# harmony-one/harmony

Hardware: AMD Instinct MI355X
Metric: BLS12-381 aggregate-verifies/sec (committee=4096) (higher is better)
Workload: dtype u64; 1 GPU; config2: committee=4096 masked aggregate + pairing verify, batch=262144/step, masks Bernoulli(0.9) seed 42, 48B staking commit payloads; parallelism=dp1 (per-shard replicas, no collective)

## Files before the change

harmony_amd/core.py:

```python
import ctypes
import os

_DIR = os.path.dirname(os.path.abspath(__file__))
_SO = os.environ.get("HBLS_SO", os.path.join(_DIR, "libhbls.so"))

HBLS_OK = 1
HBLS_FALSE = 0
HBLS_ERR = -1
HBLS_ERR_NOGPU = -2
HBLS_ERR_BADINPUT = -3
HBLS_NOQUORUM = -4
NOQUORUM = HBLS_NOQUORUM
TWO_THIRDS_DEC = 666666666666666667


class HblsError(RuntimeError):
    pass


class NoGpuError(HblsError):
    pass


class BadInputError(HblsError, ValueError):
# ... 40 lines not shown
        ctypes.c_char_p, ctypes.c_char_p, ctypes.c_size_t, ctypes.c_size_t,
        ctypes.POINTER(ctypes.c_int32)]
    lib.hbls_stream_create.restype = ctypes.c_void_p
    lib.hbls_stream_create.argtypes = [ctypes.c_void_p, ctypes.c_int]
    lib.hbls_stream_free.argtypes = [ctypes.c_void_p]
    lib.hbls_stream_set_rounds.argtypes = [
        ctypes.c_void_p, ctypes.POINTER(ctypes.c_uint32), ctypes.c_int,
        ctypes.c_char_p, ctypes.c_size_t]
    lib.hbls_stream_process.argtypes = [
        ctypes.c_void_p, ctypes.POINTER(ctypes.c_uint32),
        ctypes.POINTER(ctypes.c_uint32), ctypes.c_char_p,
        ctypes.POINTER(ctypes.c_uint32), ctypes.c_int,
        ctypes.c_size_t, ctypes.POINTER(ctypes.c_int32)]
    lib.hbls_stream_check.argtypes = [
        ctypes.c_void_p, ctypes.POINTER(ctypes.c_uint32), ctypes.c_int,
        ctypes.POINTER(ctypes.c_int32)]
    lib.hbls_stream_check_submit.argtypes = [
        ctypes.c_void_p, ctypes.POINTER(ctypes.c_uint32), ctypes.c_int]
    lib.hbls_stream_check_poll.argtypes = [
        ctypes.c_void_p, ctypes.POINTER(ctypes.c_int32)]
    lib.hbls_stream_get.argtypes = [ctypes.c_void_p, ctypes.c_uint32,
                                    ctypes.c_char_p, ctypes.c_char_p]
    lib.hbls_stream_set_verify_mode.argtypes = [ctypes.c_void_p, ctypes.c_int]
    lib.hbls_batch_verify_votes_grouped.argtypes = [
        ctypes.c_void_p, ctypes.POINTER(ctypes.c_uint32),
        ctypes.POINTER(ctypes.c_uint32), ctypes.c_char_p, ctypes.c_char_p,
        ctypes.c_size_t, ctypes.c_size_t, ctypes.c_size_t,
        ctypes.POINTER(ctypes.c_int32)]
    lib.hbls_vote_key_sums.argtypes = [
        ctypes.c_void_p, ctypes.POINTER(ctypes.c_uint32),
        ctypes.POINTER(ctypes.c_uint32), ctypes.c_size_t, ctypes.c_char_p,
        ctypes.POINTER(ctypes.c_int32)]
    lib.hbls_batch_verify_votes_multi.argtypes = [
        ctypes.c_void_p, ctypes.POINTER(ctypes.c_uint32),
        ctypes.POINTER(ctypes.c_uint32), ctypes.c_char_p, ctypes.c_char_p,
        ctypes.c_size_t, ctypes.c_size_t, ctypes.POINTER(ctypes.c_int32)]
    lib.hbls_stream_process_multi.argtypes = [
        ctypes.c_void_p, ctypes.POINTER(ctypes.c_uint32),
        ctypes.POINTER(ctypes.c_uint32), ctypes.POINTER(ctypes.c_uint32),
        ctypes.c_char_p, ctypes.POINTER(ctypes.c_uint32), ctypes.c_int,
        ctypes.c_size_t, ctypes.POINTER(ctypes.c_int32)]
    lib.hbls_rlc_last_stats.argtypes = [ctypes.POINTER(ctypes.c_uint32)]
    lib.hbls_rlc_last_stats.restype = None
    lib.hbls_set_agg_verify_mode.argtypes = [ctypes.c_int]
    lib.hbls_set_aggrlc_threshold.argtypes = [ctypes.c_int]
    lib.hbls_set_aggrlc_threshold.restype = None
    lib.hbls_aggrlc_last_stats.argtypes = [ctypes.POINTER(ctypes.c_uint32)]
    lib.hbls_aggrlc_last_stats.restype = None
    lib.hbls_set_aggrlc_final.argtypes = [ctypes.c_int]
    lib.hbls_aggrlc_final_selftest.argtypes = [ctypes.c_int]
    lib.hbls_set_aggrlc_sigleg.argtypes = [ctypes.c_int]
    lib.hbls_set_aggrlc_early.argtypes = [ctypes.c_int]
    lib.hbls_set_aggrlc_chunkleg.argtypes = [ctypes.c_int]
    lib.hbls_aggrlc_probe.argtypes = [ctypes.c_int, ctypes.c_char_p, ctypes.c_size_t,
                                      ctypes.c_char_p]
    lib.hbls_last_host_ns.restype = ctypes.c_uint64
    lib.hbls_last_host_ns.argtypes = [ctypes.c_int]
    u64p, u32p, i32p = (ctypes.POINTER(t) for t in
                        (ctypes.c_uint64, ctypes.c_uint32, ctypes.c_int32))
    lib.hbls_committee_set_quorum.argtypes = [ctypes.c_void_p, u64p, ctypes.c_uint64]
    lib.hbls_mask_power.argtypes = [ctypes.c_void_p, ctypes.c_char_p, ctypes.c_size_t,
                                    u64p, u32p]
    lib.hbls_agg_verify_quorum.argtypes = lib.hbls_agg_verify.argtypes
    lib.hbls_batch_agg_verify_quorum.argtypes = lib.hbls_batch_agg_verify.argtypes
    lib.hbls_batch_seal_verify_quorum.argtypes = lib.hbls_batch_seal_verify.argtypes
    lib.hbls_stream_power.argtypes = [ctypes.c_void_p, u32p, ctypes.c_int,
                                      u64p, u32p, i32p]
    lib.hbls_last_stage_ns.argtypes = [ctypes.c_int]
    lib.hbls_copy_bench_ns.restype = ctypes.c_uint64
    lib.hbls_copy_bench_ns.argtypes = [ctypes.c_size_t]
    lib.hbls_fpmul_bench_waves.restype = ctypes.c_double
    lib.hbls_fpmul_bench_waves.argtypes = [ctypes.c_int, ctypes.c_int]
    lib.hbls_coop_selftest.restype = ctypes.c_int
    lib.hbls_fpmul_asm_check.restype = ctypes.c_longlong
    lib.hbls_arith_probe.argtypes = [ctypes.c_int, ctypes.c_char_p, ctypes.c_size_t,
                                     ctypes.c_char_p, i32p]
    lib.hbls_arith_probe_op_name.argtypes = [ctypes.c_int]
    lib.hbls_arith_probe_op_name.restype = ctypes.c_char_p
    if hasattr(lib, "hbls_ctxset_create"):
        lib.hbls_ctxset_create.restype = ctypes.c_void_p
        lib.hbls_ctxset_create.argtypes = [ctypes.POINTER(ctypes.c_void_p), ctypes.c_size_t]
        lib.hbls_ctxset_free.argtypes = [ctypes.c_void_p]
        lib.hbls_ctxset_free.restype = None
        lib.hbls_ctxset_size.argtypes = [ctypes.c_void_p]
        lib.hbls_ctxset_size.restype = ctypes.c_size_t
        lib.hbls_batch_seal_verify_ctx.argtypes = [
            ctypes.c_void_p, u32p, ctypes.c_char_p, u32p, ctypes.c_char_p, u32p,
            ctypes.c_size_t, ctypes.c_int, i32p]
        lib.hbls_ctx_mask_sums.argtypes = [
            ctypes.c_void_p, u32p, ctypes.c_char_p, u32p, ctypes.c_size_t,
            ctypes.c_char_p, u64p, u32p, i32p]
    return lib


_lib = _load()


def _check(rc, what):
    if rc == HBLS_ERR_NOGPU:
        raise NoGpuError(f"{what}: no AMD GPU available (product path requires gfx950)")
    if rc == HBLS_ERR_BADINPUT:
        raise BadInputError(f"{what}: bad input")
    if rc < 0:
        raise HblsError(f"{what}: error {rc}")
    return rc

# ... 24 lines not shown

def set_coop_threshold(n: int):
    _lib.hbls_set_coop_threshold(n)


def rlc_chunk_size() -> int:
    return _lib.hbls_rlc_chunk_size()


def rlc_last_stats():
    out = (ctypes.c_uint32 * 4)()
    _lib.hbls_rlc_last_stats(out)
    return list(out)


def set_agg_verify_mode(mode: int):
    _check(_lib.hbls_set_agg_verify_mode(mode), "set_agg_verify_mode")


def set_aggrlc_threshold(n: int):
    _lib.hbls_set_aggrlc_threshold(n)


def aggrlc_chunk_size() -> int:
    return _lib.hbls_aggrlc_chunk_size()


def aggrlc_last_stats():
    out = (ctypes.c_uint32 * 3)()
    _lib.hbls_aggrlc_last_stats(out)
    return list(out)


def set_aggrlc_final(kernel: int):
    _check(_lib.hbls_set_aggrlc_final(kernel), "set_aggrlc_final")


def aggrlc_final_selftest(nchunks: int) -> int:
    return _check(_lib.hbls_aggrlc_final_selftest(nchunks), "aggrlc_final_selftest")


def set_aggrlc_sigleg(leg: int):
    _check(_lib.hbls_set_aggrlc_sigleg(leg), "set_aggrlc_sigleg")


def set_aggrlc_early(early: int):
    _check(_lib.hbls_set_aggrlc_early(early), "set_aggrlc_early")


def set_aggrlc_chunkleg(kernel: int):
    _check(_lib.hbls_set_aggrlc_chunkleg(kernel), "set_aggrlc_chunkleg")


AGGRLC_PROBE_OPS = {"g1_mul64w": (0, 3 * 48 + 8, 3 * 48),
                    "g2_mul64w": (1, 6 * 48 + 8, 6 * 48),
                    "miller1_fe": (2, 6 * 48, 12 * 48)}


def aggrlc_probe(name: str, data: bytes, n_items: int) -> bytes:
    op, in_b, out_b = AGGRLC_PROBE_OPS[name]
    if len(data) != n_items * in_b:
        raise ValueError("aggrlc_probe: operand size")
    out = ctypes.create_string_buffer(max(1, n_items * out_b))
    _check(_lib.hbls_aggrlc_probe(op, data, n_items, out), "aggrlc_probe")
    return out.raw[:n_items * out_b]


def last_host_ns(i: int) -> int:
    return _lib.hbls_last_host_ns(i)


def pk_from_sk(sk32: bytes) -> bytes:
    out = ctypes.create_string_buffer(48)
    _check(_lib.hbls_pk_from_sk(sk32, out), "pk_from_sk")
    return out.raw


def batch_pk_from_sk(sks: bytes, batch: int) -> bytes:
    out = ctypes.create_string_buffer(48 * batch)
    _check(_lib.hbls_batch_pk_from_sk(sks, batch, out), "batch_pk_from_sk")
    return out.raw


def sign_hash(sk32: bytes, msg: bytes) -> bytes:
    out = ctypes.create_string_buffer(96)
    _check(_lib.hbls_sign_hash(sk32, msg, len(msg), out), "sign_hash")
    return out.raw


def batch_sign(sks: bytes, msgs: bytes, mlen: int, batch: int) -> bytes:
    out = ctypes.create_string_buffer(96 * batch)
    _check(_lib.hbls_batch_sign(sks, msgs, mlen, batch, out), "batch_sign")
    return out.raw


def hash_to_g2(msg: bytes) -> bytes:
    out = ctypes.create_string_buffer(96)
    _check(_lib.hbls_hash_to_g2(msg, len(msg), out), "hash_to_g2")
    return out.raw


def batch_hash_to_g2(msgs: bytes, mlen: int, batch: int) -> bytes:
    out = ctypes.create_string_buffer(96 * batch)
    _check(_lib.hbls_batch_hash_to_g2(msgs, mlen, batch, out), "batch_hash_to_g2")
    return out.raw


def verify_hash(pk48: bytes, sig96: bytes, msg: bytes) -> bool:
    rc = _lib.hbls_verify_hash(pk48, sig96, msg, len(msg))
# ... 456 lines not shown
```

harmony_amd/csrc/hbls_aggrlc.inc:

```

#define AGGRLC_CHUNK 64
#define AGGRLC_WINDOWS 8


DEV void aggrlc_recode64(uint64_t k, uint64_t &mag, uint32_t &neg, uint32_t &top) {
    uint32_t c = 0;
    mag = 0; neg = 0;
#pragma unroll
    for (int j = 0; j < 16; j++) {
        uint32_t v = ((uint32_t)(k >> (4 * j)) & 15u) + c;
        uint32_t nx = j < 15 ? ((uint32_t)(k >> (4 * j + 4)) & 15u) : 0u;
        c = (v > 8u || (v == 8u && nx >= 8u)) ? 1u : 0u;
        uint32_t m = c ? 16u - v : v;
        mag |= (uint64_t)m << (4 * j);
        neg |= (c && m) ? (1u << j) : 0u;
    }
    top = c;
}

DEVN void g1_mul64w(g1_t &r, const g1_t &p, uint64_t k) {
    g1_t tab[8];
    tab[0] = p;
    g1_dbl(tab[1], tab[0]);
    g1_add(tab[2], tab[1], tab[0]);
// ... 196 lines not shown
__global__ void k_aggrlc_miller1(const g1_t *aggpubs, const g2_t *hms,
                                 const uint64_t *scalars, const g2aff_t *S,
                                 const int32_t *sflag, fp12_t *F, int32_t *elig,
                                 int32_t *results, int batch, int nchunks,
                                 int32_t *dirty) {
    size_t i = (size_t)blockIdx.x * blockDim.x + threadIdx.x;
    if (i >= (size_t)batch + (size_t)nchunks) return;
    fp12_t f;
    g2aff_t Q;
    g1aff_t P;
    bool run = false;
    if (i < (size_t)batch) {
        if (HOISTED) {
            int32_t e = elig[i];
            if (e == AGGRLC_ELIG_OPEN) {
                results[i] = g1_is_inf(aggpubs[i]) ? 1 : 0;
                elig[i] = 0;
            } else if (e == 1 && g1_is_inf(aggpubs[i])) {
                results[i] = 0;
                elig[i] = 0;
                dirty[i / AGGRLC_CHUNK] = 1;
            }
        }
        if (elig[i] == 1) {
            uint64_t r = scalars[i];
            if (r == 0) r = 1;
            g1_t A;
            g1_mul64w(A, aggpubs[i], r);
            if (g1_is_inf(A)) {
                elig[i] = 2; results[i] = 0;
            } else {
                g1_to_affine(P, A);
                g2_t hmc = hms[i];
                g2_to_affine(Q, hmc);
                run = true;
            }
        }
    } else {
        size_t c = i - (size_t)batch;
        if (sflag[c]) {
            Q = S[c];
            fp_load(P.x, BLS_G1_X);
            fp_t gy;
            fp_load(gy, BLS_G1_Y);
            fp_neg(P.y, gy);
            run = true;
        }
    }
    if (run) miller_loop1_h(f, Q, P);
    else fp12_one(f);
    F[i] = f;
}

__global__ void k_aggrlc_chunkleg(const g2aff_t *S, const int32_t *sflag,
                                  const int32_t *dirty, fp12_t *FX, int nchunks) {
    int c = blockIdx.x * blockDim.x + threadIdx.x;
    if (c >= nchunks) return;
    if (dirty && !dirty[c]) return;
    fp12_t f;
    if (sflag[c]) {
        g2aff_t Q = S[c];
        g1aff_t P;
        fp_load(P.x, BLS_G1_X);
        fp_t gy;
        fp_load(gy, BLS_G1_Y);
        fp_neg(P.y, gy);
        miller_loop1_h(f, Q, P);
    } else {
        fp12_one(f);
    }
    FX[c] = f;
}

DEVN void cv_miller1(lds_fp2 *A, int q) {
    if (q == 0) {
        lds_st(A + CV_T1, lds_ld(A + CV_Q1));
        lds_st(A + (CV_T1 + 1), lds_ld(A + (CV_Q1 + 1)));
        fp2_t one; fp_one(one.a); fp_zero(one.b);
        lds_st(A + (CV_T1 + 2), one);
    }
    __syncthreads();
    cv_fp12_set_one(A, q, CV_F0);
    int cur = CV_F0, oth = CV_F1;
    for (int bit = 62; bit >= 0; bit--) {
        cv_fp12_sqr(A, q, oth, cur);
        { int s = cur; cur = oth; oth = s; }
        cv_ml_dbl_step(A, q, CV_T1, CV_PP);
        cv_fp12_mul_line(A, q, oth, cur);
        { int s = cur; cur = oth; oth = s; }
        if ((BLS_U >> bit) & 1) {
            cv_ml_add_step(A, q, CV_T1, CV_Q1, CV_PP);
            cv_fp12_mul_line(A, q, oth, cur);
            { int s = cur; cur = oth; oth = s; }
        }
    }
    if (cur != CV_F0) cv_fp12_copy(A, q, CV_F0, cur);
}

template <int ITEMS>
__global__ void __launch_bounds__(ITEMS * CV_LANES) k_aggrlc_chunkleg_coop(
        const g2aff_t *S, const int32_t *sflag, fp12_t *FX, int nchunks) {
    __shared__ uint64_t arena[ITEMS][CV_STRIDE64];
    __shared__ int32_t pre[ITEMS];
    const int sub = threadIdx.x / CV_LANES;
    const int q = threadIdx.x % CV_LANES;
    const int c = blockIdx.x * ITEMS + sub;
// ... 150 lines not shown
    return HBLS_OK;
}
extern "C" void hbls_set_aggrlc_threshold(int n) {
    g_aggrlc_threshold = n < 0 ? AGGRLC_DEFAULT_THRESHOLD : n;
}

#define AGGRLC_FINAL_DEFAULT 16
static int g_aggrlc_final = -2;
static int aggrlc_final_kernel(void) {
    if (g_aggrlc_final == -2) {
        const char *e = getenv("HBLS_AGGRLC_FINAL");
        int k = e ? atoi(e) : AGGRLC_FINAL_DEFAULT;
        g_aggrlc_final = (k == 0 || k == 8 || k == 16) ? k : AGGRLC_FINAL_DEFAULT;
    }
    return g_aggrlc_final;
}
extern "C" int hbls_set_aggrlc_final(int kernel) {
    if (kernel == -1) kernel = AGGRLC_FINAL_DEFAULT;
    if (kernel != 0 && kernel != 8 && kernel != 16) return HBLS_ERR_BADINPUT;
    g_aggrlc_final = kernel;
    return HBLS_OK;
}
#define AGGRLC_SIGLEG_MIN_BATCH 16384
static int g_aggrlc_sigleg = -2;
static int aggrlc_sigleg(size_t batch) {
    if (g_aggrlc_sigleg == -2) {
        const char *e = getenv("HBLS_AGGRLC_SIGLEG");
        int k = e ? atoi(e) : -1;
        g_aggrlc_sigleg = (k == 0 || k == 1) ? k : -1;
    }
    if (g_aggrlc_sigleg >= 0) return g_aggrlc_sigleg;
    return batch >= AGGRLC_SIGLEG_MIN_BATCH ? 1 : 0;
}
extern "C" int hbls_set_aggrlc_sigleg(int leg) {
    if (leg < -1 || leg > 1) return HBLS_ERR_BADINPUT;
    g_aggrlc_sigleg = leg;
    return HBLS_OK;
}

#define AGGRLC_EARLY_MIN_BATCH 262144
static int g_aggrlc_early = -2;
static int aggrlc_early(size_t batch) {
    if (g_aggrlc_early == -2) {
        const char *e = getenv("HBLS_AGGRLC_EARLY");
        int k = e ? atoi(e) : -1;
        g_aggrlc_early = (k == 0 || k == 1) ? k : -1;
    }
    if (g_aggrlc_early >= 0) return g_aggrlc_early;
    return batch >= AGGRLC_EARLY_MIN_BATCH ? 1 : 0;
}
extern "C" int hbls_set_aggrlc_early(int early) {
    if (early < -1 || early > 1) return HBLS_ERR_BADINPUT;
    g_aggrlc_early = early;
    return HBLS_OK;
}

#define AGGRLC_CHUNKLEG_DEFAULT 16
static int g_aggrlc_chunkleg = -2;
static int aggrlc_chunkleg_kernel(void) {
    if (g_aggrlc_chunkleg == -2) {
        const char *e = getenv("HBLS_AGGRLC_CHUNKLEG");
        int k = e ? atoi(e) : AGGRLC_CHUNKLEG_DEFAULT;
        g_aggrlc_chunkleg = (k == 0 || k == 16) ? k : AGGRLC_CHUNKLEG_DEFAULT;
    }
    return g_aggrlc_chunkleg;
}
extern "C" int hbls_set_aggrlc_chunkleg(int kernel) {
    if (kernel == -1) kernel = AGGRLC_CHUNKLEG_DEFAULT;
    if (kernel != 0 && kernel != 16) return HBLS_ERR_BADINPUT;
    g_aggrlc_chunkleg = kernel;
    return HBLS_OK;
}

static hipStream_t g_aggrlc_side_stream = nullptr;
static std::once_flag g_aggrlc_side_flag;
static hipStream_t aggrlc_side_stream(void) {
    std::call_once(g_aggrlc_side_flag, [] {
        hipStream_t s = nullptr;
        int least = 0, greatest = 0;
        if (hipDeviceGetStreamPriorityRange(&least, &greatest) != hipSuccess) {
            (void)hipGetLastError();
            greatest = 0;
        }
        if (hipStreamCreateWithPriority(&s, hipStreamNonBlocking, greatest) == hipSuccess)
            g_aggrlc_side_stream = s;
        else
            (void)hipGetLastError();
    });
    return g_aggrlc_side_stream;
}

struct AggrlcEarly {
    size_t batch, nc;
    std::vector<uint64_t> scalars;
    DevBuf dsc, dB, dS, dFX, delig, dflag;
    EventSet<5> ev;
    bool launched = false;
    AggrlcEarly(size_t b, size_t n)
        : batch(b), nc(n), scalars(b), dsc(b * 8), dB(b * sizeof(g2_t)),
          dS(n * sizeof(g2aff_t)), dFX(n * sizeof(fp12_t)), delig(b * 4), dflag(2 * n * 4) {}
    bool ok() const {
        return !dsc.err && !dB.err && !dS.err && !dFX.err && !delig.err && !dflag.err &&
               ev.err == hipSuccess;
    }
    int32_t *sflag() const { return dflag.as<int32_t>(); }
    int32_t *dirty() const { return dflag.as<int32_t>() + nc; }
// ... 114 lines not shown
    std::vector<int32_t> v(3 * nc);
    HIP_OK(hipMemcpy(v.data(), dv.p, 3 * nc * 4, hipMemcpyDeviceToHost));
    int zeros = 0, ones = 0;
    for (size_t c = 0; c < nc; c++) {
        int kind = (int)(c % 8);
        int want = (kind == 1 || kind == 2 || kind == 3) ? 1 : 0;
        if (v[c] != want) return HBLS_ERR;
        if (v[c]) ones++; else zeros++;
    }
    if (nc >= 2 && (!zeros || !ones)) return HBLS_ERR;
    int diff = 0;
    for (size_t c = 0; c < nc; c++)
        if (v[nc + c] != v[c] || v[2 * nc + c] != v[c]) diff++;
    return diff;
}

static g1aff_t *g_aggrlc_gtab = nullptr;
static int aggrlc_init_tables(void) {
    if (g_aggrlc_gtab) return HBLS_OK;
    const size_t m = AGGRLC_WINDOWS * 255;
    DevBuf dp2(64 * sizeof(g1aff_t)), dwj(m * sizeof(g1_t)), dwi(m);
    g1aff_t *d_gt = nullptr;
    if (dp2.err || dwj.err || dwi.err) return HBLS_ERR;
    HIP_OK(hipMalloc(&d_gt, m * sizeof(g1aff_t)));
    hipLaunchKernelGGL(k_aggrlc_pow2, dim3(1), dim3(64), 0, 0, dp2.as<g1aff_t>());
    hipLaunchKernelGGL(k_wtab_build_jac, dim3(1), dim3(64), 0, 0,
                       dp2.as<g1aff_t>(), 64, dwj.as<g1_t>(), AGGRLC_WINDOWS);
    hipLaunchKernelGGL(k_wtab_to_affine, dim3((int)((m + 255) / 256)), dim3(256), 0, 0,
                       dwj.as<g1_t>(), d_gt, dwi.as<uint8_t>(), m);
    std::vector<uint8_t> winf(m);
    bool ok = hipDeviceSynchronize() == hipSuccess &&
              hipMemcpy(winf.data(), dwi.p, m, hipMemcpyDeviceToHost) == hipSuccess;
    for (size_t k = 0; ok && k < m; k++)
        if (winf[k]) ok = false;
    if (!ok) { hipFree(d_gt); return HBLS_ERR; }
    g_aggrlc_gtab = d_gt;
    return HBLS_OK;
}

static bool aggrlc_wanted(size_t batch) {
    int m = agg_verify_mode();
    if (m == 0 || !g_aggrlc_gtab) return false;
    if (batch > RLC_MAX_ITEMS || (long long)batch < (long long)g_aggrlc_threshold) return false;
    if (m == 1) return true;
    return (int)batch > coop_threshold() && rf_mode() == 0 && !use_batch_affine();
}

static int aggrlc_verify(const g1_t *d_agg, const g2_t *d_hm, const g2aff_t *d_saff,
                         const int32_t *d_sflags, const int32_t *d_hok,
                         int32_t *d_res, size_t batch, AggrlcEarly *early) {
    size_t nc = (batch + AGGRLC_CHUNK - 1) / AGGRLC_CHUNK;
    const int leg = early ? 1 : aggrlc_sigleg(batch);
    const size_t nx = (leg && !early) ? nc : 0;
    std::vector<uint64_t> scalars(early ? 0 : batch);
    if (!early && !rlc_draw_scalars(scalars.data(), batch)) return AGGRLC_FALLBACK;
    FreeClock fclk;
    uint64_t t_alloc = host_now_ns();
    const size_t f_bytes = (batch + nx) * sizeof(fp12_t);
    const size_t b_bytes = nx ? batch * sizeof(g2_t) : 0;
    DevBuf dsc(early ? 0 : batch * 8), dF(f_bytes + b_bytes + nx * sizeof(g2aff_t));
    DevBuf delig(early ? 0 : batch * 4);
    DevBuf dFC(nc * sizeof(fp12_t)), dcs((3 * nc + nx) * 4);
    g_host_ns[0] += host_now_ns() - t_alloc;
    FreeClockArm farm(fclk);
    if (dsc.err || dF.err || delig.err || dFC.err || dcs.err) {
        (void)hipGetLastError();
        return AGGRLC_FALLBACK;
    }
    fp12_t *d_F = dF.as<fp12_t>();
    g2_t *d_B = (g2_t *)((uint8_t *)dF.p + f_bytes);
    g2aff_t *d_S = (g2aff_t *)((uint8_t *)dF.p + f_bytes + b_bytes);
    const uint64_t *d_sc = early ? early->dsc.as<uint64_t>() : dsc.as<uint64_t>();
    int32_t *d_elig = early ? early->delig.as<int32_t>() : delig.as<int32_t>();
    EventSet<1> up;
    if (up.err != hipSuccess) return HBLS_ERR;
    if (!early) HIP_OK(upload_then_wait(dsc.p, scalars.data(), batch * 8, up[0]));
    int32_t *d_ccnt = dcs.as<int32_t>(), *d_cforce = d_ccnt + nc, *d_verdict = d_cforce + nc;
    int32_t *d_sf = d_verdict + nc;
    EventSet<5> ev;
    if (ev.err != hipSuccess) return HBLS_ERR;
    (void)hipEventRecord(ev[0], 0);
    if (leg && !early) {
        hipLaunchKernelGGL(k_aggrlc_sigscale<false>, dim3((uint32_t)((batch + 63) / 64)), dim3(64),
                           0, 0, d_agg, d_saff, d_sflags, d_hok, d_sc, d_B,
                           d_elig, d_res, (int)batch);
        hipLaunchKernelGGL(k_aggrlc_sigsum<false>, dim3((uint32_t)nc), dim3(AGGRLC_CHUNK), 0, 0,
                           d_B, (int)batch, (int)nc, d_S, d_sf,
                           (const int32_t *)nullptr, (const int32_t *)nullptr);
    }
    (void)hipEventRecord(ev[1], 0);
    if (early) {
        hipLaunchKernelGGL(k_aggrlc_miller1<true>, dim3((uint32_t)((batch + 63) / 64)), dim3(64),
                           0, 0, d_agg, d_hm, d_sc, early->dS.as<g2aff_t>(), early->sflag(), d_F,
                           d_elig, d_res, (int)batch, 0, early->dirty());
        (void)hipStreamWaitEvent(0, early->ev[3], 0);
        hipLaunchKernelGGL(k_aggrlc_sigsum<true>, dim3((uint32_t)nc), dim3(AGGRLC_CHUNK), 0, 0,
                           early->dB.as<g2_t>(), (int)batch, (int)nc, early->dS.as<g2aff_t>(),
                           early->sflag(), d_elig, early->dirty());
        hipLaunchKernelGGL(k_aggrlc_chunkleg, dim3((uint32_t)((nc + 63) / 64)), dim3(64), 0, 0,
                           early->dS.as<g2aff_t>(), early->sflag(), early->dirty(),
                           early->dFX.as<fp12_t>(), (int)nc);
    } else if (leg) {
        hipLaunchKernelGGL(k_aggrlc_miller1<false>, dim3((uint32_t)((batch + nc + 63) / 64)),
                           dim3(64), 0, 0, d_agg, d_hm, d_sc, d_S, d_sf, d_F,
                           d_elig, d_res, (int)batch, (int)nc, (int32_t *)nullptr);
    } else {
        hipLaunchKernelGGL(k_aggrlc_miller, dim3((uint32_t)((batch + 63) / 64)), dim3(64), 0, 0,
                           d_agg, d_hm, d_saff, d_sflags, d_hok, d_sc,
                           g_aggrlc_gtab, d_F, d_elig, d_res, (int)batch);
    }
    (void)hipEventRecord(ev[2], 0);
    hipLaunchKernelGGL(k_aggrlc_chunk_prod, dim3((uint32_t)nc), dim3(AGGRLC_CHUNK), 0, 0,
                       d_F, d_elig, (int)batch, (int)nc,
                       dFC.as<fp12_t>(), d_ccnt, d_cforce,
                       early ? early->dFX.as<fp12_t>()
                             : leg ? d_F + batch : (const fp12_t *)nullptr);
    (void)hipEventRecord(ev[3], 0);
    launch_aggrlc_final(aggrlc_final_kernel(), dFC.as<fp12_t>(), d_ccnt, d_cforce,
                        d_verdict, (int)nc);
    (void)hipEventRecord(ev[4], 0);
    std::vector<int32_t> hc(3 * nc);
    hipError_t e = hipMemcpy(hc.data(), dcs.p, 3 * nc * 4, hipMemcpyDeviceToHost);
    if (e == hipSuccess) e = hipGetLastError();
    for (int i = 0; i < 4; i++) {
        float ms = 0;
        if (e == hipSuccess && (i || (leg && !early)))
            (void)hipEventElapsedTime(&ms, ev[i], ev[i + 1]);
        g_stage_ns[i ? 3 + i : 7] = (uint64_t)(ms * 1e6);
    }
    if (early && e == hipSuccess) {
        float ms = 0;
        (void)hipEventElapsedTime(&ms, early->ev[0], early->ev[1]);
        g_stage_ns[7] = (uint64_t)(ms * 1e6);
        ms = 0;
        (void)hipEventElapsedTime(&ms, early->ev[2], early->ev[3]);
        g_stage_ns[8] = (uint64_t)(ms * 1e6);
    }
    HIP_OK(e);

    std::vector<uint32_t> failed;
    for (size_t c = 0; c < nc; c++) {
        if (hc[c] <= 0) continue;
        g_aggrlc_stats[0]++;
        if (hc[2 * nc + c] == 1) continue;
        g_aggrlc_stats[1]++;
        failed.push_back((uint32_t)c);
    }
    if (failed.empty()) return HBLS_OK;

    std::vector<int32_t> helig(batch);
    HIP_OK(hipMemcpy(helig.data(), d_elig, batch * 4, hipMemcpyDeviceToHost));
    std::vector<uint32_t> sel;
    for (uint32_t c : failed)
        for (size_t i = (size_t)c * AGGRLC_CHUNK;
             i < batch && i < ((size_t)c + 1) * AGGRLC_CHUNK; i++)
            if (helig[i]) sel.push_back((uint32_t)i);
    size_t ns = sel.size();
    g_aggrlc_stats[2] = (uint32_t)ns;
    if (!ns) return HBLS_OK;
    DevBuf dsel(ns * 4);
    if (dsel.err) return HBLS_ERR;
    HIP_OK(hipMemcpy(dsel.p, sel.data(), ns * 4, hipMemcpyHostToDevice));
    hipLaunchKernelGGL(k_verify_sel, dim3((uint32_t)((ns + 63) / 64)), dim3(64), 0, 0,
                       dsel.as<uint32_t>(), (int)ns, d_agg, d_hm, d_saff, d_sflags, d_hok,
                       d_res, (int)batch);
    HIP_OK(hipGetLastError());
    return HBLS_OK;
}

enum { AGGRLC_PROBE_G1_MUL64W = 0, AGGRLC_PROBE_G2_MUL64W = 1, AGGRLC_PROBE_MILLER1_FE = 2,
       AGGRLC_PROBE_N_OPS = 3 };
#define AGGRLC_PROBE_MAX_ITEMS 4096
__global__ void k_aggrlc_probe(int op, const uint64_t *in, int in_w, uint64_t *out, int out_w,
                               int n) {
    int j = blockIdx.x * blockDim.x + threadIdx.x;
    if (j >= n) return;
    const uint64_t *src = in + (size_t)j * in_w;
    uint64_t *dst = out + (size_t)j * out_w;
    union { uint64_t w[72]; g1_t g1; g2_t g2; g2aff_t q; fp12_t f; } a, o;
    for (int i = 0; i < in_w && i < 72; i++) a.w[i] = src[i];
    if (op == AGGRLC_PROBE_G1_MUL64W) {
        g1_mul64w(o.g1, a.g1, src[18]);
    } else if (op == AGGRLC_PROBE_G2_MUL64W) {
        g2_mul64w(o.g2, a.g2, src[36]);
    } else {
        g1aff_t p;
        for (int k = 0; k < 6; k++) { p.x.l[k] = src[24 + k]; p.y.l[k] = src[30 + k]; }
        fp12_t f;
        miller_loop1_h(f, a.q, p);
        fp12_conj(f, f);
        final_exp(o.f, f);
    }
    for (int i = 0; i < out_w; i++) dst[i] = o.w[i];
}
static bool probe_limbs_lt_p(const uint8_t *b);
extern "C" int hbls_aggrlc_probe(int op, const uint8_t *in, size_t n_items, uint8_t *out) {
    if (op < 0 || op >= AGGRLC_PROBE_N_OPS) return HBLS_ERR_BADINPUT;
    if (!in || !out || n_items == 0 || n_items > AGGRLC_PROBE_MAX_ITEMS)
        return HBLS_ERR_BADINPUT;
    const int n_fp = op == AGGRLC_PROBE_G1_MUL64W ? 3 : 6;
    const int in_w = n_fp * 6 + (op == AGGRLC_PROBE_MILLER1_FE ? 0 : 1);
    const int out_w = op == AGGRLC_PROBE_G1_MUL64W ? 18 : op == AGGRLC_PROBE_G2_MUL64W ? 36 : 72;
    for (size_t j = 0; j < n_items; j++)
        for (int i = 0; i < n_fp; i++)
            if (!probe_limbs_lt_p(in + j * (size_t)in_w * 8 + 48 * i)) return HBLS_ERR_BADINPUT;
    int rc = require_gpu();
    if (rc != HBLS_OK) return rc;
    DevBuf din(n_items * in_w * 8), dout(n_items * out_w * 8);
    if (din.err || dout.err) return HBLS_ERR;
    HIP_OK(hipMemcpy(din.p, in, n_items * in_w * 8, hipMemcpyHostToDevice));
    hipLaunchKernelGGL(k_aggrlc_probe, dim3((uint32_t)((n_items + 63) / 64)), dim3(64), 0, 0,
                       op, din.as<uint64_t>(), in_w, dout.as<uint64_t>(), out_w, (int)n_items);
    HIP_OK(hipGetLastError());
    HIP_OK(hipDeviceSynchronize());
    HIP_OK(hipMemcpy(out, dout.p, n_items * out_w * 8, hipMemcpyDeviceToHost));
    return HBLS_OK;
}
```

harmony_amd/csrc/hbls_dev.hip:

```cpp
#include <hip/hip_runtime.h>
#include <stdint.h>
#include <string.h>
#include <stdio.h>
#include <stdlib.h>
#include "../../oracle/bls_consts.h"
#include "../../include/hbls.h"

typedef unsigned __int128 u128;

#define DEV __device__ __forceinline__
#define DEVN __device__ __noinline__

struct fp_t { uint64_t l[6]; };
struct fp2_t { fp_t a, b; };

DEV bool fp_is_zero(const fp_t &x) {
    return (x.l[0] | x.l[1] | x.l[2] | x.l[3] | x.l[4] | x.l[5]) == 0;
}
DEV bool fp_eq(const fp_t &x, const fp_t &y) {
    uint64_t d = 0;
#pragma unroll
    for (int i = 0; i < 6; i++) d |= x.l[i] ^ y.l[i];
    return d == 0;
}
// ... 1088 lines not shown
    fp2_dbl(E, E); fp2_dbl(E, E);
    fp2_dbl(t, E); fp2_add(E, E, t);
    fp2_dbl(t, E); fp2_add(F, E, t);
    fp2_add(G, B, F);
    fp2_half(G, G);
    fp2_add(H, T.y, T.z);
    fp2_sqr(H, H);
    fp2_add(t, B, C);
    fp2_sub(H, H, t);
    fp2_sqr(XX, T.x);
    fp2_mul_fp(t, H, Pa.y);
    fp2_mul_xi(c0, t);
    fp2_sub(c3, B, E);
    fp2_dbl(t, XX); fp2_add(t, t, XX);
    fp2_mul_fp(t, t, Pa.x);
    fp2_neg(c5, t);
    fp2_sub(t, B, F);
    fp2_mul(T.x, A, t);
    fp2_sqr(t, G);
    fp2_sqr(t2, E);
    fp2_dbl(G, t2); fp2_add(t2, t2, G);
    fp2_sub(T.y, t, t2);
    fp2_mul(T.z, B, H);
}
DEVN void ml_add_step_h(g2_t &T, const g2aff_t &Q, const g1aff_t &Pa,
                        fp2_t &c0, fp2_t &c3, fp2_t &c5) {
    fp2_t th, la, C, D, E, F, G, H, t, t2;
    fp2_mul(t, Q.y, T.z);
    fp2_sub(th, T.y, t);
    fp2_mul(t, Q.x, T.z);
    fp2_sub(la, T.x, t);
    fp2_mul_fp(t, la, Pa.y);
    fp2_mul_xi(c0, t);
    fp2_mul(t, Q.x, th);
    fp2_mul(t2, Q.y, la);
    fp2_sub(c3, t, t2);
    fp2_mul_fp(t, th, Pa.x);
    fp2_neg(c5, t);
    fp2_sqr(C, th);
    fp2_sqr(D, la);
    fp2_mul(E, la, D);
    fp2_mul(F, T.z, C);
    fp2_mul(G, T.x, D);
    fp2_add(H, E, F);
    fp2_dbl(t, G);
    fp2_sub(H, H, t);
    fp2_mul(T.x, la, H);
    fp2_sub(t, G, H);
    fp2_mul(t, th, t);
    fp2_mul(t2, E, T.y);
    fp2_sub(T.y, t, t2);
    fp2_mul(T.z, T.z, E);
}
DEVN void fp12_mul_line2(fp12_t &f, const fp2_t &a0, const fp2_t &a3, const fp2_t &a5,
                         const fp2_t &b0, const fp2_t &b3, const fp2_t &b5) {
    fp6_t m0, t0, t1, fs, tt, vt1;
    fp2_t p00, p33, p55, x, y, s, u, q1, q2, q3;
    fp2_mul(p00, a0, b0);
    fp2_mul(p33, a3, b3);
    fp2_mul(p55, a5, b5);
    fp2_add(s, a3, a5);
    fp2_add(u, b3, b5);
    fp2_mul(q1, s, u);
    fp2_sub(q1, q1, p33);
    fp2_sub(q1, q1, p55);
    fp2_mul_xi(m0.c1, q1);
    fp2_mul_xi(s, p33);
    fp2_add(m0.c0, p00, s);
    fp2_mul_xi(m0.c2, p55);
    fp2_add(s, a0, a3);
    fp2_add(u, b0, b3);
    fp2_mul(x, s, u);
    fp2_sub(x, x, p00);
    fp2_sub(x, x, p33);
    fp2_add(s, a0, a5);
    fp2_add(u, b0, b5);
    fp2_mul(y, s, u);
    fp2_sub(y, y, p00);
    fp2_sub(y, y, p55);
    fp6_mul(t0, f.c0, m0);
    {
        const fp2_t &g0 = f.c1.c0, &g1 = f.c1.c1, &g2 = f.c1.c2;
        fp2_mul(q1, g1, x);
        fp2_mul(q2, g2, y);
        fp2_add(s, g1, g2);
        fp2_add(u, x, y);
        fp2_mul(q3, s, u);
        fp2_sub(q3, q3, q1);
        fp2_sub(q3, q3, q2);
        fp2_mul_xi(t1.c0, q3);
        fp2_mul(s, g0, x);
        fp2_mul_xi(u, q2);
        fp2_add(t1.c1, s, u);
        fp2_mul(s, g0, y);
        fp2_add(t1.c2, s, q1);
    }
    fp6_add(fs, f.c0, f.c1);
    fp2_add(m0.c1, m0.c1, x);
    fp2_add(m0.c2, m0.c2, y);
    fp6_mul(tt, fs, m0);
    fp6_sub(tt, tt, t0);
    fp6_sub(tt, tt, t1);
    fp6_mul_v(vt1, t1);
    fp6_add(f.c0, t0, vt1);
    f.c1 = tt;
}
// ... 2988 lines not shown
```

include/hbls.h:

```cpp
#ifndef HBLS_H
#define HBLS_H

#include <stddef.h>
#include <stdint.h>

#ifdef __cplusplus
extern "C" {
#endif

enum {
    HBLS_OK = 1,
    HBLS_FALSE = 0,
    HBLS_ERR = -1,
    HBLS_ERR_NOGPU = -2,
    HBLS_ERR_BADINPUT = -3,
    HBLS_NOQUORUM = -4,
};

#define HBLS_TWO_THIRDS_DEC 666666666666666667ULL

int hbls_init(int device);

int hbls_device_count(void);

// ... 104 lines not shown
                               const uint8_t *msgs,  const uint32_t *msg_off,
                               size_t batch, int quorum, int32_t *results);

int hbls_ctx_mask_sums(const hbls_ctxset_t *s, const uint32_t *ctx_idx,
                       const uint8_t *bitmaps, const uint32_t *bm_off, size_t batch,
                       uint8_t *out48s, uint64_t *power_out, uint32_t *count_out,
                       int32_t *ok);

int hbls_g2_aggregate(const uint8_t *sigs96, size_t n, uint8_t out96[96]);

typedef struct hbls_stream hbls_stream_t;
hbls_stream_t *hbls_stream_create(const hbls_committee_t *c, int max_rounds);
void hbls_stream_free(hbls_stream_t *s);
int hbls_stream_set_rounds(hbls_stream_t *s, const uint32_t *slots, int k,
                           const uint8_t *payloads, size_t payload_len);
int hbls_stream_process(hbls_stream_t *s, const uint32_t *key_idx,
                        const uint32_t *round_idx, const uint8_t *sigs96,
                        const uint32_t *active_slots, int n_active,
                        size_t batch, int32_t *results);
int hbls_stream_set_verify_mode(hbls_stream_t *s, int mode);
int hbls_stream_check(hbls_stream_t *s, const uint32_t *slots, int k, int32_t *ok);
int hbls_stream_check_submit(hbls_stream_t *s, const uint32_t *slots, int k);
int hbls_stream_check_poll(hbls_stream_t *s, int32_t *ok);
int hbls_stream_get(hbls_stream_t *s, uint32_t slot, uint8_t *bitmap_out,
                    uint8_t agg96_out[96]);

int hbls_stream_power(hbls_stream_t *s, const uint32_t *slots, int k,
                      uint64_t *power_out, uint32_t *count_out, int32_t *quorum_out);


int hbls_vote_key_sums(const hbls_committee_t *c, const uint32_t *key_off,
                       const uint32_t *key_idx, size_t batch,
                       uint8_t *out48s, int32_t *ok);

int hbls_batch_verify_votes_multi(const hbls_committee_t *c, const uint32_t *key_off,
                                  const uint32_t *key_idx, const uint8_t *sigs96,
                                  const uint8_t *msgs, size_t msg_len, size_t batch,
                                  int32_t *results);

int hbls_stream_process_multi(hbls_stream_t *s, const uint32_t *key_off,
                              const uint32_t *key_idx, const uint32_t *round_idx,
                              const uint8_t *sigs96, const uint32_t *active_slots,
                              int n_active, size_t batch, int32_t *results);

int hbls_set_agg_verify_mode(int mode);
void hbls_set_aggrlc_threshold(int min_batch);
int hbls_aggrlc_chunk_size(void);
void hbls_aggrlc_last_stats(uint32_t out[3]);
int hbls_set_aggrlc_final(int kernel);
int hbls_aggrlc_final_selftest(int nchunks);
int hbls_set_aggrlc_sigleg(int leg);
int hbls_set_aggrlc_early(int early);
int hbls_set_aggrlc_chunkleg(int kernel);

int hbls_batch_keccak256(const uint8_t *msgs, size_t msg_len, size_t batch,
                         uint8_t *out32s);

const char *hbls_version(void);
double hbls_mad_peak_ops(void);
uint64_t hbls_last_kernel_ns(void);
uint64_t hbls_last_host_ns(int i);

#ifdef __cplusplus
}
#endif
#endif
```

Before: 806,700 aggregate-verifies/sec.

## Use projective-input Miller loop and fuse chunk product into wave shuffles

Adds a Miller loop variant that takes the scaled G1 point and hashed G2 point in projective form, so per-item affine normalization and its inversions are skipped. Adds a fused kernel where each 64-lane wavefront multiplies its Fp12 Miller outputs together with cross-lane shuffles and Karatsuba role splitting. Each chunk then writes one partial product instead of writing every per-item Fp12 value to global memory and launching a separate chunk-product kernel. A small fold kernel multiplies in the signature-leg values. This is enabled by default at level 2. It costs extra shuffle traffic and register pressure, and it adds a new correctness surface in the lane-role arithmetic.

```diff
diff --git a/harmony_amd/core.py b/harmony_amd/core.py
--- a/harmony_amd/core.py
+++ b/harmony_amd/core.py
@@ -116,6 +116,7 @@
     lib.hbls_set_aggrlc_sigleg.argtypes = [ctypes.c_int]
     lib.hbls_set_aggrlc_early.argtypes = [ctypes.c_int]
     lib.hbls_set_aggrlc_chunkleg.argtypes = [ctypes.c_int]
+    lib.hbls_set_aggrlc_miller.argtypes = [ctypes.c_int]
     lib.hbls_aggrlc_probe.argtypes = [ctypes.c_int, ctypes.c_char_p, ctypes.c_size_t,
                                       ctypes.c_char_p]
     lib.hbls_last_host_ns.restype = ctypes.c_uint64
@@ -246,9 +247,15 @@
     _check(_lib.hbls_set_aggrlc_chunkleg(kernel), "set_aggrlc_chunkleg")
 
 
+def set_aggrlc_miller(level: int):
+    _check(_lib.hbls_set_aggrlc_miller(level), "set_aggrlc_miller")
+
+
 AGGRLC_PROBE_OPS = {"g1_mul64w": (0, 3 * 48 + 8, 3 * 48),
                     "g2_mul64w": (1, 6 * 48 + 8, 6 * 48),
-                    "miller1_fe": (2, 6 * 48, 12 * 48)}
+                    "miller1_fe": (2, 6 * 48, 12 * 48),
+                    "miller1j_fe": (3, 9 * 48, 12 * 48),
+                    "wave_prod": (4, 64 * 12 * 48, 2 * 12 * 48)}
 
 
 def aggrlc_probe(name: str, data: bytes, n_items: int) -> bytes:
diff --git a/harmony_amd/csrc/hbls_aggrlc.inc b/harmony_amd/csrc/hbls_aggrlc.inc
--- a/harmony_amd/csrc/hbls_aggrlc.inc
+++ b/harmony_amd/csrc/hbls_aggrlc.inc
@@ -272,6 +272,123 @@
     F[i] = f;
 }
 
+DEVN void fp12_wave_prod(fp12_t &f) {
+    union { fp12_t v; uint32_t w[144]; } a, b;
+    union { fp6_t v; uint32_t w[72]; } u, t0, t1, tt;
+    a.v = f;
+#pragma unroll
+    for (int i = 0; i < 144; i++) b.w[i] = (uint32_t)__shfl_xor((int)a.w[i], 1, 64);
+    fp12_mul(a.v, a.v, b.v);
+    const int lane = (int)(threadIdx.x & 63u), role = lane & 3, quad = lane & ~3;
+    for (int m = 2; m < 64; m <<= 1) {
+#pragma unroll
+        for (int i = 0; i < 144; i++) b.w[i] = (uint32_t)__shfl_xor((int)a.w[i], m, 64);
+        fp6_t p, q;
+        fp6_add(p, a.v.c0, a.v.c1);
+        fp6_add(q, b.v.c0, b.v.c1);
+        if (role == 0) { p = a.v.c0; q = b.v.c0; }
+        if (role == 1) { p = a.v.c1; q = b.v.c1; }
+        fp6_mul(u.v, p, q);
+#pragma unroll
+        for (int i = 0; i < 72; i++) {
+            t0.w[i] = (uint32_t)__shfl((int)u.w[i], quad, 64);
+            t1.w[i] = (uint32_t)__shfl((int)u.w[i], quad + 1, 64);
+            tt.w[i] = (uint32_t)__shfl((int)u.w[i], quad + 2, 64);
+        }
+        fp6_sub(tt.v, tt.v, t0.v);
+        fp6_sub(a.v.c1, tt.v, t1.v);
+        fp6_mul_v(u.v, t1.v);
+        fp6_add(a.v.c0, t0.v, u.v);
+    }
+    f = a.v;
+}
+
+template <bool HOISTED, bool FUSED>
+__global__ void k_aggrlc_miller1j(const g1_t *aggpubs, const g2_t *hms,
+                                  const uint64_t *scalars, const g2aff_t *S,
+                                  const int32_t *sflag, fp12_t *F, int32_t *elig,
+                                  int32_t *results, int batch, int nchunks,
+                                  int32_t *dirty, fp12_t *FC, int32_t *ccnt,
+                                  int32_t *cforce) {
+    const bool item_block = !FUSED || (int)blockIdx.x < nchunks;
+    size_t i = (size_t)blockIdx.x * blockDim.x + threadIdx.x;
+    size_t c = 0;
+    bool is_item, is_entry;
+    if (FUSED) {
+        is_item = item_block && i < (size_t)batch;
+        c = i - (size_t)nchunks * blockDim.x;
+        is_entry = !HOISTED && !item_block && c < (size_t)nchunks;
+        if (!item_block && !is_entry) return;
+    } else {
+        if (i >= (size_t)batch + (size_t)nchunks) return;
+        is_item = i < (size_t)batch;
+        is_entry = !is_item;
+        c = i - (size_t)batch;
+    }
+    fp12_t f;
+    int32_t e = 0;
+    bool run = false;
+    if (is_item) {
+        e = elig[i];
+        if (HOISTED) {
+            if (e == AGGRLC_ELIG_OPEN) {
+                results[i] = g1_is_inf(aggpubs[i]) ? 1 : 0;
+                elig[i] = e = 0;
+            } else if (e == 1 && g1_is_inf(aggpubs[i])) {
+                results[i] = 0;
+                elig[i] = e = 0;
+                dirty[i / AGGRLC_CHUNK] = 1;
+            }
+        }
+        if (e == 1) {
+            uint64_t r = scalars[i];
+            if (r == 0) r = 1;
+            g1_t A;
+            g1_mul64w(A, aggpubs[i], r);
+            g2_t hmc = hms[i];
+            if (g1_is_inf(A) || g2_is_inf(hmc)) {
+                elig[i] = e = 2; results[i] = 0;
+            } else {
+                miller_loop1_hj(f, hmc, A);
+                run = true;
+            }
+        }
+    } else if (!HOISTED && is_entry) {
+        if (sflag[c]) {
+            g2aff_t Q = S[c];
+            g1aff_t P;
+            fp_load(P.x, BLS_G1_X);
+            fp_t gy;
+            fp_load(gy, BLS_G1_Y);
+            fp_neg(P.y, gy);
+            miller_loop1_h(f, Q, P);
+            run = true;
+        }
+    }
+    if (!run) fp12_one(f);
+    if (!FUSED) {
+        F[i] = f;
+    } else if (!item_block) {
+        F[c] = f;
+    } else {
+        fp12_wave_prod(f);
+        unsigned long long any = __ballot(e != 0), force = __ballot(e == 2);
+        if (threadIdx.x == 0) {
+            FC[blockIdx.x] = f;
+            ccnt[blockIdx.x] = __popcll(any);
+            cforce[blockIdx.x] = force ? 1 : 0;
+        }
+    }
+}
+
+__global__ void k_aggrlc_chunk_fold(fp12_t *FC, const fp12_t *FX, int nchunks) {
+    int c = blockIdx.x * blockDim.x + threadIdx.x;
+    if (c >= nchunks) return;
+    fp12_t a = FC[c], b = FX[c];
+    fp12_mul(a, a, b);
+    FC[c] = a;
+}
+
 __global__ void k_aggrlc_chunkleg(const g2aff_t *S, const int32_t *sflag,
                                   const int32_t *dirty, fp12_t *FX, int nchunks) {
     int c = blockIdx.x * blockDim.x + threadIdx.x;
@@ -528,6 +645,22 @@
 extern "C" int hbls_set_aggrlc_early(int early) {
     if (early < -1 || early > 1) return HBLS_ERR_BADINPUT;
     g_aggrlc_early = early;
+    return HBLS_OK;
+}
+
+#define AGGRLC_MILLER_DEFAULT 2
+static int g_aggrlc_miller = -2;
+static int aggrlc_miller_level(void) {
+    if (g_aggrlc_miller == -2) {
+        const char *e = getenv("HBLS_AGGRLC_MILLER");
+        bool digit = e && e[0] >= '0' && e[0] <= '2' && e[1] == '\0';
+        g_aggrlc_miller = digit ? e[0] - '0' : AGGRLC_MILLER_DEFAULT;
+    }
+    return g_aggrlc_miller;
+}
+extern "C" int hbls_set_aggrlc_miller(int level) {
+    if (level < -1 || level > 2) return HBLS_ERR_BADINPUT;
+    g_aggrlc_miller = level == -1 ? AGGRLC_MILLER_DEFAULT : level;
     return HBLS_OK;
 }
 
@@ -748,11 +881,14 @@
     size_t nc = (batch + AGGRLC_CHUNK - 1) / AGGRLC_CHUNK;
     const int leg = early ? 1 : aggrlc_sigleg(batch);
     const size_t nx = (leg && !early) ? nc : 0;
+    const int lvl = leg ? aggrlc_miller_level() : 0;
+    const bool fused = lvl == 2;
     std::vector<uint64_t> scalars(early ? 0 : batch);
     if (!early && !rlc_draw_scalars(scalars.data(), batch)) return AGGRLC_FALLBACK;
     FreeClock fclk;
     uint64_t t_alloc = host_now_ns();
-    const size_t f_bytes = (batch + nx) * sizeof(fp12_t);
+    const size_t nf = fused ? 0 : batch;
+    const size_t f_bytes = (nf + nx) * sizeof(fp12_t);
     const size_t b_bytes = nx ? batch * sizeof(g2_t) : 0;
     DevBuf dsc(early ? 0 : batch * 8), dF(f_bytes + b_bytes + nx * sizeof(g2aff_t));
     DevBuf delig(early ? 0 : batch * 4);
@@ -786,9 +922,21 @@
     }
     (void)hipEventRecord(ev[1], 0);
     if (early) {
-        hipLaunchKernelGGL(k_aggrlc_miller1<true>, dim3((uint32_t)((batch + 63) / 64)), dim3(64),
-                           0, 0, d_agg, d_hm, d_sc, early->dS.as<g2aff_t>(), early->sflag(), d_F,
-                           d_elig, d_res, (int)batch, 0, early->dirty());
+        if (fused)
+            hipLaunchKernelGGL((k_aggrlc_miller1j<true, true>), dim3((uint32_t)nc), dim3(64),
+                               0, 0, d_agg, d_hm, d_sc, early->dS.as<g2aff_t>(), early->sflag(),
+                               d_F, d_elig, d_res, (int)batch, (int)nc, early->dirty(),
+                               dFC.as<fp12_t>(), d_ccnt, d_cforce);
+        else if (lvl == 1)
+            hipLaunchKernelGGL((k_aggrlc_miller1j<true, false>),
+                               dim3((uint32_t)((batch + 63) / 64)), dim3(64),
+                               0, 0, d_agg, d_hm, d_sc, early->dS.as<g2aff_t>(), early->sflag(),
+                               d_F, d_elig, d_res, (int)batch, 0, early->dirty(),
+                               (fp12_t *)nullptr, (int32_t *)nullptr, (int32_t *)nullptr);
+        else
+            hipLaunchKernelGGL(k_aggrlc_miller1<true>, dim3((uint32_t)((batch + 63) / 64)),
+                               dim3(64), 0, 0, d_agg, d_hm, d_sc, early->dS.as<g2aff_t>(),
+                               early->sflag(), d_F, d_elig, d_res, (int)batch, 0, early->dirty());
         (void)hipStreamWaitEvent(0, early->ev[3], 0);
         hipLaunchKernelGGL(k_aggrlc_sigsum<true>, dim3((uint32_t)nc), dim3(AGGRLC_CHUNK), 0, 0,
                            early->dB.as<g2_t>(), (int)batch, (int)nc, early->dS.as<g2aff_t>(),
@@ -796,6 +944,17 @@
         hipLaunchKernelGGL(k_aggrlc_chunkleg, dim3((uint32_t)((nc + 63) / 64)), dim3(64), 0, 0,
                            early->dS.as<g2aff_t>(), early->sflag(), early->dirty(),
                            early->dFX.as<fp12_t>(), (int)nc);
+    } else if (fused) {
+        hipLaunchKernelGGL((k_aggrlc_miller1j<false, true>),
+                           dim3((uint32_t)(nc + (nc + 63) / 64)), dim3(64), 0, 0, d_agg, d_hm,
+                           d_sc, d_S, d_sf, d_F, d_elig, d_res, (int)batch, (int)nc,
+                           (int32_t *)nullptr, dFC.as<fp12_t>(), d_ccnt, d_cforce);
+    } else if (lvl == 1) {
+        hipLaunchKernelGGL((k_aggrlc_miller1j<false, false>),
+                           dim3((uint32_t)((batch + nc + 63) / 64)), dim3(64), 0, 0, d_agg, d_hm,
+                           d_sc, d_S, d_sf, d_F, d_elig, d_res, (int)batch, (int)nc,
+                           (int32_t *)nullptr, (fp12_t *)nullptr, (int32_t *)nullptr,
+                           (int32_t *)nullptr);
     } else if (leg) {
         hipLaunchKernelGGL(k_aggrlc_miller1<false>, dim3((uint32_t)((batch + nc + 63) / 64)),
                            dim3(64), 0, 0, d_agg, d_hm, d_sc, d_S, d_sf, d_F,
@@ -806,11 +965,15 @@
                            g_aggrlc_gtab, d_F, d_elig, d_res, (int)batch);
     }
     (void)hipEventRecord(ev[2], 0);
-    hipLaunchKernelGGL(k_aggrlc_chunk_prod, dim3((uint32_t)nc), dim3(AGGRLC_CHUNK), 0, 0,
-                       d_F, d_elig, (int)batch, (int)nc,
-                       dFC.as<fp12_t>(), d_ccnt, d_cforce,
-                       early ? early->dFX.as<fp12_t>()
-                             : leg ? d_F + batch : (const fp12_t *)nullptr);
+    const fp12_t *d_FX = early ? early->dFX.as<fp12_t>()
+                               : leg ? d_F + nf : (const fp12_t *)nullptr;
+    if (fused)
+        hipLaunchKernelGGL(k_aggrlc_chunk_fold, dim3((uint32_t)((nc + 63) / 64)), dim3(64), 0, 0,
+                           dFC.as<fp12_t>(), d_FX, (int)nc);
+    else
+        hipLaunchKernelGGL(k_aggrlc_chunk_prod, dim3((uint32_t)nc), dim3(AGGRLC_CHUNK), 0, 0,
+                           d_F, d_elig, (int)batch, (int)nc,
+                           dFC.as<fp12_t>(), d_ccnt, d_cforce, d_FX);
     (void)hipEventRecord(ev[3], 0);
     launch_aggrlc_final(aggrlc_final_kernel(), dFC.as<fp12_t>(), d_ccnt, d_cforce,
                         d_verdict, (int)nc);
@@ -865,7 +1028,8 @@
 }
 
 enum { AGGRLC_PROBE_G1_MUL64W = 0, AGGRLC_PROBE_G2_MUL64W = 1, AGGRLC_PROBE_MILLER1_FE = 2,
-       AGGRLC_PROBE_N_OPS = 3 };
+       AGGRLC_PROBE_MILLER1J_FE = 3, AGGRLC_PROBE_WAVE_PROD = 4, AGGRLC_PROBE_N_OPS = 5 };
+#define AGGRLC_PROBE_MAX_GROUPS 64
 #define AGGRLC_PROBE_MAX_ITEMS 4096
 __global__ void k_aggrlc_probe(int op, const uint64_t *in, int in_w, uint64_t *out, int out_w,
                                int n) {
@@ -879,6 +1043,15 @@
         g1_mul64w(o.g1, a.g1, src[18]);
     } else if (op == AGGRLC_PROBE_G2_MUL64W) {
         g2_mul64w(o.g2, a.g2, src[36]);
+    } else if (op == AGGRLC_PROBE_MILLER1J_FE) {
+        g1_t p;
+        for (int k = 0; k < 6; k++) {
+            p.x.l[k] = src[36 + k]; p.y.l[k] = src[42 + k]; p.z.l[k] = src[48 + k];
+        }
+        fp12_t f;
+        miller_loop1_hj(f, a.g2, p);
+        fp12_conj(f, f);
+        final_exp(o.f, f);
     } else {
         g1aff_t p;
         for (int k = 0; k < 6; k++) { p.x.l[k] = src[24 + k]; p.y.l[k] = src[30 + k]; }
@@ -889,14 +1062,27 @@
     }
     for (int i = 0; i < out_w; i++) dst[i] = o.w[i];
 }
+__global__ void k_aggrlc_probe_wave_prod(const fp12_t *in, fp12_t *out, int n) {
+    int g = blockIdx.x;
+    if (g >= n) return;
+    fp12_t f = in[(size_t)g * 64 + threadIdx.x];
+    fp12_wave_prod(f);
+    if (threadIdx.x == 0) out[2 * g] = f;
+    if (threadIdx.x == 63) out[2 * g + 1] = f;
+}
 static bool probe_limbs_lt_p(const uint8_t *b);
 extern "C" int hbls_aggrlc_probe(int op, const uint8_t *in, size_t n_items, uint8_t *out) {
     if (op < 0 || op >= AGGRLC_PROBE_N_OPS) return HBLS_ERR_BADINPUT;
     if (!in || !out || n_items == 0 || n_items > AGGRLC_PROBE_MAX_ITEMS)
         return HBLS_ERR_BADINPUT;
-    const int n_fp = op == AGGRLC_PROBE_G1_MUL64W ? 3 : 6;
-    const int in_w = n_fp * 6 + (op == AGGRLC_PROBE_MILLER1_FE ? 0 : 1);
-    const int out_w = op == AGGRLC_PROBE_G1_MUL64W ? 18 : op == AGGRLC_PROBE_G2_MUL64W ? 36 : 72;
+    const bool wave = op == AGGRLC_PROBE_WAVE_PROD;
+    if (wave && n_items > AGGRLC_PROBE_MAX_GROUPS) return HBLS_ERR_BADINPUT;
+    const bool mul = op == AGGRLC_PROBE_G1_MUL64W || op == AGGRLC_PROBE_G2_MUL64W;
+    const int n_fp = op == AGGRLC_PROBE_G1_MUL64W ? 3 : op == AGGRLC_PROBE_MILLER1J_FE ? 9
+                     : wave ? 64 * 12 : 6;
+    const int in_w = n_fp * 6 + (mul ? 1 : 0);
+    const int out_w = op == AGGRLC_PROBE_G1_MUL64W ? 18 : op == AGGRLC_PROBE_G2_MUL64W ? 36
+                      : wave ? 144 : 72;
     for (size_t j = 0; j < n_items; j++)
         for (int i = 0; i < n_fp; i++)
             if (!probe_limbs_lt_p(in + j * (size_t)in_w * 8 + 48 * i)) return HBLS_ERR_BADINPUT;
@@ -905,8 +1091,12 @@
     DevBuf din(n_items * in_w * 8), dout(n_items * out_w * 8);
     if (din.err || dout.err) return HBLS_ERR;
     HIP_OK(hipMemcpy(din.p, in, n_items * in_w * 8, hipMemcpyHostToDevice));
-    hipLaunchKernelGGL(k_aggrlc_probe, dim3((uint32_t)((n_items + 63) / 64)), dim3(64), 0, 0,
-                       op, din.as<uint64_t>(), in_w, dout.as<uint64_t>(), out_w, (int)n_items);
+    if (wave)
+        hipLaunchKernelGGL(k_aggrlc_probe_wave_prod, dim3((uint32_t)n_items), dim3(64), 0, 0,
+                           din.as<fp12_t>(), dout.as<fp12_t>(), (int)n_items);
+    else
+        hipLaunchKernelGGL(k_aggrlc_probe, dim3((uint32_t)((n_items + 63) / 64)), dim3(64), 0, 0,
+                           op, din.as<uint64_t>(), in_w, dout.as<uint64_t>(), out_w, (int)n_items);
     HIP_OK(hipGetLastError());
     HIP_OK(hipDeviceSynchronize());
     HIP_OK(hipMemcpy(out, dout.p, n_items * out_w * 8, hipMemcpyDeviceToHost));
diff --git a/harmony_amd/csrc/hbls_dev.hip b/harmony_amd/csrc/hbls_dev.hip
--- a/harmony_amd/csrc/hbls_dev.hip
+++ b/harmony_amd/csrc/hbls_dev.hip
@@ -1164,6 +1164,67 @@
     fp2_sub(T.y, t, t2);
     fp2_mul(T.z, T.z, E);
 }
+DEVN void ml_add_step_hj(g2_t &T, const g2_t &Q2, const g1aff_t &Pp, const fp_t &k,
+                         fp2_t &c0, fp2_t &c3, fp2_t &c5) {
+    fp2_t th, la, yz, xz, zz, C, D, E, F, G, H, t, t2;
+    fp2_mul(yz, T.y, Q2.z);
+    fp2_mul(t, Q2.y, T.z);
+    fp2_sub(th, yz, t);
+    fp2_mul(xz, T.x, Q2.z);
+    fp2_mul(t, Q2.x, T.z);
+    fp2_sub(la, xz, t);
+    fp2_mul(zz, T.z, Q2.z);
+    fp2_mul(t, la, Q2.z);
+    fp2_mul_fp(t, t, Pp.y);
+    fp2_mul_xi(c0, t);
+    fp2_mul(t, Q2.x, th);
+    fp2_mul(t2, Q2.y, la);
+    fp2_sub(t, t, t2);
+    fp2_mul_fp(c3, t, k);
+    fp2_mul(t, th, Q2.z);
+    fp2_mul_fp(t, t, Pp.x);
+    fp2_neg(c5, t);
+    fp2_sqr(C, th);
+    fp2_sqr(D, la);
+    fp2_mul(E, la, D);
+    fp2_mul(F, zz, C);
+    fp2_mul(G, xz, D);
+    fp2_add(H, E, F);
+    fp2_dbl(t, G);
+    fp2_sub(H, H, t);
+    fp2_mul(T.x, la, H);
+    fp2_sub(t, G, H);
+    fp2_mul(t, th, t);
+    fp2_mul(t2, E, yz);
+    fp2_sub(T.y, t, t2);
+    fp2_mul(T.z, zz, E);
+}
+DEVN void miller_loop1_hj(fp12_t &f, const g2_t &Qj, const g1_t &Pj) {
+    g1aff_t Pp;
+    fp_t k;
+    fp_sqr(k, Pj.z);
+    fp_mul(k, k, Pj.z);
+    fp_mul(Pp.x, Pj.x, Pj.z);
+    Pp.y = Pj.y;
+    g2_t Q2, T;
+    fp2_t c0, c3, c5;
+    fp2_sqr(c0, Qj.z);
+    fp2_mul(Q2.z, c0, Qj.z);
+    fp2_mul(Q2.x, Qj.x, Qj.z);
+    Q2.y = Qj.y;
+    T = Q2;
+    fp12_one(f);
+    for (int bit = 62; bit >= 0; bit--) {
+        fp12_sqr(f, f);
+        ml_dbl_step_h(T, Pp, c0, c3, c5);
+        fp2_mul_fp(c3, c3, k);
+        fp12_mul_line(f, c0, c3, c5);
+        if ((BLS_U >> bit) & 1) {
+            ml_add_step_hj(T, Q2, Pp, k, c0, c3, c5);
+            fp12_mul_line(f, c0, c3, c5);
+        }
+    }
+}
 DEVN void fp12_mul_line2(fp12_t &f, const fp2_t &a0, const fp2_t &a3, const fp2_t &a5,
                          const fp2_t &b0, const fp2_t &b3, const fp2_t &b5) {
     fp6_t m0, t0, t1, fs, tt, vt1;
diff --git a/include/hbls.h b/include/hbls.h
--- a/include/hbls.h
+++ b/include/hbls.h
@@ -180,6 +180,7 @@
 int hbls_set_aggrlc_sigleg(int leg);
 int hbls_set_aggrlc_early(int early);
 int hbls_set_aggrlc_chunkleg(int kernel);
+int hbls_set_aggrlc_miller(int level);
 
 int hbls_batch_keccak256(const uint8_t *msgs, size_t msg_len, size_t batch,
                          uint8_t *out32s);
```

Result: faster. 833,300 aggregate-verifies/sec, median of 6 (+3.3%).
